# kakaobrain/hqtransformer

Measured on AMD Instinct MI355X. Metric: images/sec (256x256 class-cond sampling), higher is better.
Workload: dtype bf16

## Files before the change

hqtransformer_amd/csrc/split_ring.h:

```cpp
#pragma once
#include "split_kernels.h"
#include "split_device.h"

typedef _Float16 half8 __attribute__((ext_vector_type(8)));
typedef __attribute__((ext_vector_type(16))) float f32x16;
typedef __attribute__((ext_vector_type(4))) float f32x4;
typedef __attribute__((ext_vector_type(4))) unsigned int u32x4;

namespace {
constexpr float R_INV = 1.0f / 2048.0f;
constexpr int R_TY = 8, R_TX = 16, R_PITCH = R_TX + 2;
constexpr int R_ROWS = (R_TY + 2) * R_PITCH;
constexpr int R_PIECES = (R_ROWS + 15) / 16;
constexpr int R_PPW = 2 * R_PIECES / 4;
constexpr int R_CPITCH = 128 * 4 + 16;
static_assert(R_PPW == 6, "one piece per wave at taps 0..5");
constexpr int G_PITCH = 80, G_PLANE = 16 * R_PIECES * G_PITCH, G_LDS = 4 * G_PLANE;
static_assert(64 * R_CPITCH <= G_LDS, "epilogue staging (64 pixels at a time) must fit in the patch buffers");
static_assert(3 * G_PLANE + 38 * G_PITCH + 32 < 65536, "ds_read immediate offsets");

constexpr int H_RING = 3, H_AHEAD = H_RING - 1, H_STEPS = 18;
static_assert(H_STEPS % H_RING == 0, "static ring slots");
constexpr bool h_piece_at(int u) { u = ((u % H_STEPS) + H_STEPS) % H_STEPS; return (u % 9) < 6; }
constexpr int h_younger(int s, int per_step = 4) {
    int n = per_step * (H_AHEAD - 1);
    for (int u = s - H_AHEAD; u < s; ++u) n += h_piece_at(u) ? 1 : 0;
    return n;
}

__device__ __forceinline__ void r_xcd_tile(int& tile_m, int& tile_n, int panel) {
    const int nx = gridDim.x, total = gridDim.x * gridDim.y;
    int id = blockIdx.x + nx * blockIdx.y;
    if ((total & 7) == 0) id = (id & 7) * (total >> 3) + (id >> 3);
    if (panel > 0) {
        const int per = panel * nx, p = id / per, r = id - p * per;
        const int rows = min(panel, (int)gridDim.y - p * panel);
        tile_n = r / rows;
        tile_m = p * panel + (r - tile_n * rows);
        return;
    }
    tile_m = id / nx;
    tile_n = id - tile_m * nx;
}

__device__ __forceinline__ void ring_tile(int tile_m, int H, int W, int& img, int& trem, int& ty0, int& tx0, int& tiles_x, int& tiles_y) {
    tiles_x = W / R_TX; tiles_y = H / R_TY;
    img = tile_m / (tiles_x * tiles_y);
    trem = tile_m - img * (tiles_x * tiles_y);
    ty0 = (trem / tiles_x) * R_TY; tx0 = (trem % tiles_x) * R_TX;
}

typedef int ring_rsrc_t __attribute__((ext_vector_type(4)));
__device__ __forceinline__ ring_rsrc_t ring_image_rsrc(const void* A, int img, int Hin, int Win, int Cin) {
    const unsigned long long ib = (unsigned long long)(size_t)(reinterpret_cast<const half_t*>(A) + (long long)img * Hin * Win * (2 * Cin));
    ring_rsrc_t rsrc;
    rsrc[0] = __builtin_amdgcn_readfirstlane((int)(unsigned)ib);
    rsrc[1] = __builtin_amdgcn_readfirstlane((int)(unsigned)(ib >> 32) & 0xffff);
    rsrc[2] = __builtin_amdgcn_readfirstlane(Hin * Win * 2 * Cin * 2);
    rsrc[3] = 0x00020000;
    return rsrc;
}
__device__ __forceinline__ void ring_piece_offsets(unsigned (&poff)[3], int wave, int lane, int ty0, int tx0, int H, int W, int Win, int up, int Cin) {
#pragma unroll
    for (int u = 0; u < 3; ++u) {
        const int piece = wave + 4 * u;
        const int q = piece * 16 + (lane >> 2);
        const int qy = (q * 3641) >> 16, qx = q - qy * R_PITCH;
        const int iy = ty0 + qy - 1, ix = tx0 + qx - 1;
        const bool in = (q < R_ROWS) & ((unsigned)iy < (unsigned)H) & ((unsigned)ix < (unsigned)W);
        const unsigned off = (unsigned)((((iy >> up) * Win + (ix >> up)) * (2 * Cin) + (lane & 3) * 8) * 2);
        poff[u] = in ? off : 0x80000000u;
    }
}
__device__ __forceinline__ unsigned ring_piece_base(unsigned lds_base, int wave, int lane) {
    return lds_base + wave * (16 * G_PITCH) + (lane >> 2) * G_PITCH + (lane & 3) * 16;
}
__device__ __forceinline__ unsigned ring_frag_base(unsigned lds_base, int row, int fk) { return lds_base + row * G_PITCH + fk * 16; }

__device__ __forceinline__ void ring_load_piece(u32x4& dst, const unsigned (&poff)[3], const ring_rsrc_t& rsrc, int c, int u, int Cin) {
    asm volatile("buffer_load_dwordx4 %0, %1, %2, %3 offen" : "=v"(dst) : "v"(poff[u % 3]), "s"(rsrc), "s"(c * 64 + (u / 3) * Cin * 2));
}
__device__ __forceinline__ void ring_store_piece(unsigned piece_base, const u32x4& src, int buf, int u) {
    asm volatile("ds_write_b128 %0, %1 offset:%2" :: "v"(piece_base), "v"(src), "n"((buf * 2 + u / 3) * G_PLANE + 4 * (u % 3) * 16 * G_PITCH) : "memory");
}
__device__ __forceinline__ void ring_read_a16(half8 (&ah)[4], half8 (&al)[4], unsigned abase, int ps, int tapoff, int i, int slot) {
    asm volatile("ds_read_b128 %0, %1 offset:%2" : "=v"(ah[slot]) : "v"(abase), "n"(ps * 2 * G_PLANE + (i * R_PITCH + tapoff) * G_PITCH));
    asm volatile("ds_read_b128 %0, %1 offset:%2" : "=v"(al[slot]) : "v"(abase), "n"(ps * 2 * G_PLANE + (i * R_PITCH + tapoff) * G_PITCH + G_PLANE));
}
__device__ __forceinline__ void ring_read_a16(half8 (&ah)[4], half8 (&al)[4], unsigned abase, int ps, int tapoff, int i) {
    ring_read_a16(ah, al, abase, ps, tapoff, i, i % 4);
}
__device__ __forceinline__ void ring_load_b4(half8 (&wh)[2], half8 (&wl)[2], unsigned lane16, const char* bfrag, long long S) {
    const char* p = bfrag + S * 4096;
    asm volatile("global_load_dwordx4 %0, %1, %2" : "=v"(wh[0]) : "v"(lane16), "s"(p));
    asm volatile("global_load_dwordx4 %0, %1, %2 offset:1024" : "=v"(wl[0]) : "v"(lane16), "s"(p));
    asm volatile("global_load_dwordx4 %0, %1, %2 offset:2048" : "=v"(wh[1]) : "v"(lane16), "s"(p));
    asm volatile("global_load_dwordx4 %0, %1, %2 offset:3072" : "=v"(wl[1]) : "v"(lane16), "s"(p));
}
__device__ __forceinline__ void ring_load_b2(half8& wh, half8& wl, unsigned lane16, const char* bfrag, long long S) {
    const char* p = bfrag + S * 4096;
    asm volatile("global_load_dwordx4 %0, %1, %2" : "=v"(wh) : "v"(lane16), "s"(p));
    asm volatile("global_load_dwordx4 %0, %1, %2 offset:1024" : "=v"(wl) : "v"(lane16), "s"(p));
}

template <class V, int NI, int NJ>
__device__ __forceinline__ void ring_sink_acc(const GemmArgs& g, const V (&accm)[NI][NJ], const V (&accx)[NI][NJ]) {
    float sacc = 0.0f;
#pragma unroll
    for (int i = 0; i < NI; ++i)
#pragma unroll
        for (int j = 0; j < NJ; ++j)
#pragma unroll
            for (int r = 0; r < (int)(sizeof(V) / sizeof(float)); ++r) sacc += accm[i][j][r] + accx[i][j][r];
    if (sacc == 12345.678f) reinterpret_cast<float*>(g.C)[0] = sacc;
}

__device__ __forceinline__ void ring_bias8(const GemmArgs& g, int nn, float (&bv)[8]) {
#pragma unroll
    for (int e = 0; e < 8; ++e) bv[e] = (g.bias && nn + e < g.N) ? g.bias[nn + e] : 0.0f;
}
template <int PASSES, bool OUT_SPLIT, class PixelOf>
__device__ __forceinline__ void ring_store_rows(const GemmArgs& g, const char* stage, int tid, int n0, const float (&bv)[8], bool active,
                                                PixelOf pixel_of, float (&gs)[8], float (&gq)[8], bool& bad) {
    float* Cb = reinterpret_cast<float*>(g.C);
    const float* Rb = reinterpret_cast<const float*>(g.resid);
    const int c8 = (tid & 15) * 8, nn = n0 + c8;
    if (active && nn < g.N) {
        long long moff[PASSES];
        f32x4 r0[PASSES], r1[PASSES];
#pragma unroll
        for (int pass = 0; pass < PASSES; ++pass) {
            const int r = pass * 16 + (tid >> 4);
            moff[pass] = pixel_of(r) * g.ldc + nn;
            if (Rb) { r0[pass] = *reinterpret_cast<const f32x4*>(Rb + moff[pass]); r1[pass] = *reinterpret_cast<const f32x4*>(Rb + moff[pass] + 4); }
        }
#pragma unroll
        for (int pass = 0; pass < PASSES; ++pass) {
            const int r = pass * 16 + (tid >> 4);
            const f32x4 lo = *reinterpret_cast<const f32x4*>(stage + r * R_CPITCH + c8 * 4);
            const f32x4 hi = *reinterpret_cast<const f32x4*>(stage + r * R_CPITCH + c8 * 4 + 16);
            float v[8] = {lo[0], lo[1], lo[2], lo[3], hi[0], hi[1], hi[2], hi[3]};
#pragma unroll
            for (int e = 0; e < 8; ++e) v[e] = v[e] * g.alpha + bv[e];
            if (Rb) {
#pragma unroll
                for (int e = 0; e < 4; ++e) { v[e] += r0[pass][e]; v[4 + e] += r1[pass][e]; }
            }
            if (OUT_SPLIT && g.out_split) {
                unsigned hi[4], lo[4];
                split8_checked(v, hi, lo, bad);
                half_t* P = reinterpret_cast<half_t*>(g.C) + 2 * moff[pass] - nn;
                *reinterpret_cast<u32x4*>(P) = u32x4{hi[0], hi[1], hi[2], hi[3]};
                *reinterpret_cast<u32x4*>(P + g.N) = u32x4{lo[0], lo[1], lo[2], lo[3]};
            } else {
                const f32x4 o0 = {v[0], v[1], v[2], v[3]}, o1 = {v[4], v[5], v[6], v[7]};
                *reinterpret_cast<f32x4*>(Cb + moff[pass]) = o0;
                *reinterpret_cast<f32x4*>(Cb + moff[pass] + 4) = o1;
            }
            if (g.gn_part_out_d) {
#pragma clang fp contract(off)
#pragma unroll
                for (int e = 0; e < 8; ++e) { gs[e] += v[e]; const float sq = v[e] * v[e]; gq[e] += sq; }
            }
        }
    }
}
template <int PASSES, class PixelOf>
__device__ __forceinline__ void ring_store_rows(const GemmArgs& g, const char* stage, int tid, int n0, const float (&bv)[8], bool active,
                                                PixelOf pixel_of, float (&gs)[8], float (&gq)[8]) {
    bool bad = false;
    ring_store_rows<PASSES, false>(g, stage, tid, n0, bv, active, pixel_of, gs, gq, bad);
}
__device__ __forceinline__ void ring_reduce_gn(const GemmArgs& g, char* lds_raw, int tid, const float (&gs)[8], const float (&gq)[8], int n0,
                                               bool active, long long part) {
    if (!g.gn_part_out_d) return;
    const int c8 = (tid & 15) * 8;
    __syncthreads();
    float* redw = reinterpret_cast<float*>(lds_raw);
    if (active) {
#pragma unroll
        for (int e = 0; e < 8; ++e) {
            redw[(((tid >> 4) * 128) + c8 + e) * 2] = gs[e];
            redw[(((tid >> 4) * 128) + c8 + e) * 2 + 1] = gq[e];
        }
    }
    __syncthreads();
    const float* red = reinterpret_cast<const float*>(lds_raw);
    if (active && tid < 128) {
        double sa = 0.0, sq = 0.0;
#pragma unroll
        for (int rg = 0; rg < 16; ++rg) { sa += (double)red[((rg * 128) + tid) * 2]; sq += (double)red[((rg * 128) + tid) * 2 + 1]; }
        const int cpg = g.N / g.gn_out_groups;
        for (int off = cpg >> 1; off > 0; off >>= 1) { sa += __shfl_xor(sa, off, 64); sq += __shfl_xor(sq, off, 64); }
        const int ch = n0 + tid;
        if (ch < g.N && (tid & (cpg - 1)) == 0) {
            double* pp = g.gn_part_out_d + (part * g.gn_out_groups + ch / cpg) * 2;
            pp[0] = sa; pp[1] = sq;
        }
    }
}
}
```

hqtransformer_amd/csrc/split_stream_conv.hip:

```cpp
#include "split_kernels.h"
#include "split_ring.h"
#include "gemm_generic.h"
#include <algorithm>
#include <cstdlib>
#include <type_traits>

constexpr size_t R_FRAG_PAD = 3 * 4 * 512;
size_t split_frag_elems(int N, int Cin) { return (size_t)((N + 31) / 32) * (Cin / 32) * 9 * 4 * 512 + R_FRAG_PAD; }

__global__ void pack_split_frag16_kernel(const float* __restrict__ w, half_t* __restrict__ out, int N, int Cin, size_t total) {
    const int NC = Cin / 32;
    for (size_t i = blockIdx.x * (size_t)blockDim.x + threadIdx.x; i < total; i += (size_t)gridDim.x * blockDim.x) {
        const int j = (int)(i & 7), lane = (int)((i >> 3) & 63);
        size_t ch = i >> 9;
        const int plane = (int)(ch & 1); ch >>= 1;
        const int blk = (int)(ch & 1); ch >>= 1;
        const int tap = (int)(ch % 9); ch /= 9;
        const int c = (int)(ch % NC);
        const int t = (int)(ch / NC);
        const int n = t * 32 + blk * 16 + (lane & 15), k = tap * Cin + c * 32 + 8 * (lane >> 4) + j;
        const float x = n < N ? w[(size_t)n * 9 * Cin + k] : 0.0f;
        const half_t hi = (half_t)x;
        out[i] = plane ? (half_t)((x - (float)hi) * 2048.0f) : hi;
    }
}
hipError_t launch_pack_split_frag16(const float* w_tapmajor, half_t* out, int N, int Cin, hipStream_t st) {
    const size_t total = split_frag_elems(N, Cin) - R_FRAG_PAD;
    pack_split_frag16_kernel<<<(int)std::min<size_t>((total + 255) / 256, 8192), 256, 0, st>>>(w_tapmajor, out, N, Cin, total);
    return hipGetLastError();
}

namespace {
__device__ __forceinline__ void h_stage_half(char* stage, const f32x4 (&accm)[8][2], const f32x4 (&accx)[8][2], int half, int wave, int fx, int fk) {
#pragma unroll
    for (int ii = 0; ii < 4; ++ii) {
        const int i = half * 4 + ii, r = ii * 16 + fx;
#pragma unroll
        for (int j = 0; j < 2; ++j) {
            const int nl = wave * 32 + j * 16 + 4 * fk;
            f32x4 v;
#pragma unroll
            for (int e = 0; e < 4; ++e) v[e] = accm[i][j][e] + accx[i][j][e] * R_INV;
            *reinterpret_cast<f32x4*>(stage + r * R_CPITCH + nl * 4) = v;
        }
    }
}
}

template <int ABL = 0>
__global__ __launch_bounds__(256, 2) void conv3x3_split_ring16_kernel(GemmArgs g) {
    constexpr int NI = 8;
    extern __shared__ __attribute__((aligned(16))) char lds_raw[];
    const unsigned lds_base = (unsigned)(size_t)(__attribute__((address_space(3))) char*)lds_raw;
    const int tid = threadIdx.x, lane = tid & 63;
    const int wave = __builtin_amdgcn_readfirstlane(tid >> 6);
    const int fx = lane & 15, fk = lane >> 4;
    int tile_m, tile_n;
    r_xcd_tile(tile_m, tile_n, g.tile_panel);
    const int n0 = tile_n * 128;
    int img, trem, ty0, tx0, tiles_x, tiles_y;
    ring_tile(tile_m, g.H, g.W, img, trem, ty0, tx0, tiles_x, tiles_y);
    const int Hin = g.H >> g.upsample, Win = g.W >> g.upsample;
    const int NC = g.Cin / 32;

    const ring_rsrc_t img_rsrc = ring_image_rsrc(g.A, img, Hin, Win, g.Cin);
    unsigned poff[3];
    ring_piece_offsets(poff, wave, lane, ty0, tx0, g.H, g.W, Win, g.upsample, g.Cin);
    u32x4 pst[2];
    unsigned piece_base = ring_piece_base(lds_base, wave, lane);

    const char* bfrag = reinterpret_cast<const char*>(reinterpret_cast<const half_t*>(g.Bw_frag16) + (size_t)(n0 / 32 + wave) * ((size_t)NC * 9 * 2048));
    unsigned lane16 = lane * 16;

    f32x4 accm[NI][2], accx[NI][2];
#pragma unroll
    for (int i = 0; i < NI; ++i)
#pragma unroll
        for (int j = 0; j < 2; ++j)
#pragma unroll
            for (int r = 0; r < 4; ++r) { accm[i][j][r] = 0.0f; accx[i][j][r] = 0.0f; }
    const unsigned abase = ring_frag_base(lds_base, fx, fk);
    half8 ah[4], al[4];
    half8 wh[H_RING][2], wl[H_RING][2];

#pragma unroll
    for (int rnd = 0; rnd < 3; ++rnd) {
        ring_load_piece(pst[0], poff, img_rsrc, 0, 2 * rnd, g.Cin); ring_load_piece(pst[1], poff, img_rsrc, 0, 2 * rnd + 1, g.Cin);
        asm volatile("s_waitcnt vmcnt(0)" : "+v"(pst[0]), "+v"(pst[1]));
        ring_store_piece(piece_base, pst[0], 0, 2 * rnd); ring_store_piece(piece_base, pst[1], 0, 2 * rnd + 1);
    }
#pragma unroll
    for (int s = 0; s < H_AHEAD; ++s) ring_load_b4(wh[s], wl[s], lane16, bfrag, s);
    asm volatile("s_waitcnt vmcnt(0) lgkmcnt(0)" ::: "memory");

#pragma unroll 1
    for (int c0 = 0; c0 < NC; c0 += 2) {
#pragma unroll
        for (int cc = 0; cc < 2; ++cc) {
            const int c = c0 + cc, cn = min(c + 1, NC - 1);
            __builtin_amdgcn_s_barrier();
            __builtin_amdgcn_sched_barrier(0);
            if (ABL != 4) { ring_read_a16(ah, al, abase, cc, 0, 0); ring_read_a16(ah, al, abase, cc, 0, 1); ring_read_a16(ah, al, abase, cc, 0, 2); ring_read_a16(ah, al, abase, cc, 0, 3); }
#pragma unroll
            for (int tap = 0; tap < 9; ++tap) {
                const int s = cc * 9 + tap, slot = s % H_RING, nslot = (s + H_AHEAD) % H_RING;
                const long long S = (long long)c0 * 9 + s;
                const int tapoff = (tap / 3) * R_PITCH + tap % 3, ntapoff = ((tap + 1) / 3) * R_PITCH + (tap + 1) % 3;
                if (ABL != 4) asm volatile("s_waitcnt vmcnt(%4)" : "+v"(wh[slot][0]), "+v"(wl[slot][0]), "+v"(wh[slot][1]), "+v"(wl[slot][1]) : "n"(h_younger(s)));
#pragma unroll
                for (int pr = 0; pr < 4; ++pr) {
                    const int i0 = 2 * pr, i1 = 2 * pr + 1;
                    if (ABL != 4) {
                        const bool more = !(tap == 8 && pr == 3);
                        if (more) asm volatile("s_waitcnt lgkmcnt(4)" : "+v"(ah[i0 % 4]), "+v"(al[i0 % 4]), "+v"(ah[i1 % 4]), "+v"(al[i1 % 4]));
                        else asm volatile("s_waitcnt lgkmcnt(0)" : "+v"(ah[i0 % 4]), "+v"(al[i0 % 4]), "+v"(ah[i1 % 4]), "+v"(al[i1 % 4]));
                    }
#pragma unroll
                    for (int ii = 0; ii < 2; ++ii)
#pragma unroll
                        for (int j = 0; j < 2; ++j)
                            accm[i0 + ii][j] = __builtin_amdgcn_mfma_f32_16x16x32_f16(wh[slot][j], ah[(i0 + ii) % 4], accm[i0 + ii][j], 0, 0, 0);
#pragma unroll
                    for (int ii = 0; ii < 2; ++ii)
#pragma unroll
                        for (int j = 0; j < 2; ++j)
                            accx[i0 + ii][j] = __builtin_amdgcn_mfma_f32_16x16x32_f16(wh[slot][j], al[(i0 + ii) % 4], accx[i0 + ii][j], 0, 0, 0);
#pragma unroll
                    for (int ii = 0; ii < 2; ++ii)
#pragma unroll
                        for (int j = 0; j < 2; ++j)
                            accx[i0 + ii][j] = __builtin_amdgcn_mfma_f32_16x16x32_f16(wl[slot][j], ah[(i0 + ii) % 4], accx[i0 + ii][j], 0, 0, 0);
                    if (ABL == 4) continue;
                    if (pr < 2) {
                        if (pr == 0) { ring_read_a16(ah, al, abase, cc, tapoff, 4); ring_read_a16(ah, al, abase, cc, tapoff, 5); }
                        else { ring_read_a16(ah, al, abase, cc, tapoff, 6); ring_read_a16(ah, al, abase, cc, tapoff, 7); }
                    } else if (tap < 8) {
                        if (pr == 2) { ring_read_a16(ah, al, abase, cc, ntapoff, 0); ring_read_a16(ah, al, abase, cc, ntapoff, 1); }
                        else { ring_read_a16(ah, al, abase, cc, ntapoff, 2); ring_read_a16(ah, al, abase, cc, ntapoff, 3); }
                    }
                    if (pr == 0 && ABL != 5) ring_load_b4(wh[nslot], wl[nslot], lane16, bfrag, S + H_AHEAD);
                    if (pr == 1 && ABL != 2) {
                        if (tap >= 2 && tap - 2 < R_PPW) {
                            if (tap - 1 < R_PPW) asm volatile("s_waitcnt vmcnt(9)" : "+v"(pst[tap % 2]));
                            else asm volatile("s_waitcnt vmcnt(8)" : "+v"(pst[tap % 2]));
                            ring_store_piece(piece_base, pst[tap % 2], cc ^ 1, tap - 2);
                        }
                        if (tap < R_PPW) ring_load_piece(pst[tap % 2], poff, img_rsrc, cn, tap, g.Cin);
                    }
                }
            }
        }
    }
    asm volatile("s_waitcnt vmcnt(0) lgkmcnt(0)" ::: "memory");
    __builtin_amdgcn_s_barrier();
    __builtin_amdgcn_sched_barrier(0);
    if (ABL == 1) { ring_sink_acc(g, accm, accx); return; }
    const long long pix0 = ((long long)img * g.H + ty0) * g.W + tx0;
    char* stage = lds_raw;
    float bv[8], gs[8], gq[8];
    ring_bias8(g, n0 + (tid & 15) * 8, bv);
    bool bad = false;
#pragma unroll
    for (int e = 0; e < 8; ++e) { gs[e] = 0.0f; gq[e] = 0.0f; }
#pragma unroll
    for (int half = 0; half < 2; ++half) {
        if (half > 0) __syncthreads();
        h_stage_half(stage, accm, accx, half, wave, fx, fk);
        __syncthreads();
        ring_store_rows<4, true>(g, stage, tid, n0, bv, true, [&](int r) { return pix0 + (long long)(half * 4 + (r >> 4)) * g.W + (r & 15); }, gs, gq, bad);
    }
    if (bad && g.range_flag) atomicOr(g.range_flag, 1);
    ring_reduce_gn(g, lds_raw, tid, gs, gq, n0, true, (long long)img * (tiles_x * tiles_y) + trem);
}


__global__ void pack_split_up16_kernel(const float* __restrict__ w, half_t* __restrict__ out, int N, int Cin, size_t total) {
    const int NC = Cin / 32, NG = (N + 31) / 32;
    for (size_t i = blockIdx.x * (size_t)blockDim.x + threadIdx.x; i < total; i += (size_t)gridDim.x * blockDim.x) {
        const int j = (int)(i & 7), lane = (int)((i >> 3) & 63);
        size_t ch = i >> 9;
        const int plane = (int)(ch & 1); ch >>= 1;
        const int blk = (int)(ch & 1); ch >>= 1;
        const int tap = (int)(ch & 3); ch >>= 2;
        const int c = (int)(ch % NC); ch /= NC;
        const int t = (int)(ch % NG);
        const int phase = (int)(ch / NG);
        const int pa = phase >> 1, pb = phase & 1, ty = tap >> 1, tx = tap & 1;
        const int n = t * 32 + blk * 16 + (lane & 15), kin = c * 32 + 8 * (lane >> 4) + j;
        const int ky0 = pa == 0 ? (ty == 0 ? 0 : 1) : (ty == 0 ? 0 : 2), ky1 = pa == 0 ? (ty == 0 ? 0 : 2) : (ty == 0 ? 1 : 2);
        const int kx0 = pb == 0 ? (tx == 0 ? 0 : 1) : (tx == 0 ? 0 : 2), kx1 = pb == 0 ? (tx == 0 ? 0 : 2) : (tx == 0 ? 1 : 2);
        double x = 0.0;
        if (n < N)
            for (int ky = ky0; ky <= ky1; ++ky)
                for (int kx = kx0; kx <= kx1; ++kx) x += (double)w[(size_t)n * 9 * Cin + (size_t)(ky * 3 + kx) * Cin + kin];
        const half_t hi = (half_t)(float)x;
        out[i] = plane ? (half_t)(float)((x - (double)(float)hi) * 2048.0) : hi;
    }
}
size_t split_up_elems(int N, int Cin) { return (size_t)4 * ((N + 31) / 32) * (Cin / 32) * 4 * 2048 + 2048; }
hipError_t launch_pack_split_up16(const float* w_tapmajor, half_t* out, int N, int Cin, hipStream_t st) {
    const size_t total = split_up_elems(N, Cin) - 2048;
    pack_split_up16_kernel<<<(int)std::min<size_t>((total + 255) / 256, 8192), 256, 0, st>>>(w_tapmajor, out, N, Cin, total);
    return hipGetLastError();
}

template <int ABL = 0>
__global__ __launch_bounds__(256, 2) void conv2x2_split_up16_kernel(GemmArgs g) {
    constexpr int NI = 8, TAPS = 4;
    extern __shared__ __attribute__((aligned(16))) char lds_raw[];
    const unsigned lds_base = (unsigned)(size_t)(__attribute__((address_space(3))) char*)lds_raw;
    const int tid = threadIdx.x, lane = tid & 63;
    const int wave = __builtin_amdgcn_readfirstlane(tid >> 6);
    const int fx = lane & 15, fk = lane >> 4;
    int tile_m, tile_v;
    r_xcd_tile(tile_m, tile_v, g.tile_panel);
    const int NT = g.N / 128;
    const int phase = tile_v / NT, pa = phase >> 1, pb = phase & 1;
    const int n0 = (tile_v - phase * NT) * 128;
    const int Hin = g.H >> 1, Win = g.W >> 1;
    int img, trem, ty0, tx0, tiles_x, tiles_y;
    ring_tile(tile_m, Hin, Win, img, trem, ty0, tx0, tiles_x, tiles_y);
    const int NC = g.Cin / 32;

    const ring_rsrc_t img_rsrc = ring_image_rsrc(g.A, img, Hin, Win, g.Cin);
    unsigned poff[3];
    ring_piece_offsets(poff, wave, lane, ty0, tx0, Hin, Win, Win, 0, g.Cin);
    u32x4 pst[R_PPW];
    unsigned piece_base = ring_piece_base(lds_base, wave, lane);

    const char* bfrag = reinterpret_cast<const char*>(reinterpret_cast<const half_t*>(g.Bw_up16) +
                                                      ((size_t)phase * (g.N / 32) + n0 / 32 + wave) * ((size_t)NC * TAPS * 2048));
    unsigned lane16 = lane * 16;

    f32x4 accm[NI][2], accx[NI][2];
#pragma unroll
    for (int i = 0; i < NI; ++i)
#pragma unroll
        for (int j = 0; j < 2; ++j)
#pragma unroll
            for (int r = 0; r < 4; ++r) { accm[i][j][r] = 0.0f; accx[i][j][r] = 0.0f; }
    const unsigned abase = ring_frag_base(lds_base, fx + pa * R_PITCH + pb, fk);
    half8 ah[4], al[4];
    half8 wh[2][2], wl[2][2];

#pragma unroll
    for (int u = 0; u < R_PPW; ++u) ring_load_piece(pst[u], poff, img_rsrc, 0, u, g.Cin);
    asm volatile("s_waitcnt vmcnt(0)" : "+v"(pst[0]), "+v"(pst[1]), "+v"(pst[2]), "+v"(pst[3]), "+v"(pst[4]), "+v"(pst[5]));
#pragma unroll
    for (int u = 0; u < R_PPW; ++u) ring_store_piece(piece_base, pst[u], 0, u);
    ring_load_b4(wh[0], wl[0], lane16, bfrag, 0);
    asm volatile("s_waitcnt vmcnt(0) lgkmcnt(0)" ::: "memory");

#pragma unroll 1
    for (int c0 = 0; c0 < NC; c0 += 2) {
#pragma unroll
        for (int cc = 0; cc < 2; ++cc) {
            const int c = c0 + cc, cn = min(c + 1, NC - 1);
            __builtin_amdgcn_s_barrier();
            __builtin_amdgcn_sched_barrier(0);
            if (ABL != 4) { ring_read_a16(ah, al, abase, cc, 0, 0); ring_read_a16(ah, al, abase, cc, 0, 1); ring_read_a16(ah, al, abase, cc, 0, 2); ring_read_a16(ah, al, abase, cc, 0, 3); }
#pragma unroll
            for (int tap = 0; tap < TAPS; ++tap) {
                const int s = cc * TAPS + tap, slot = s % 2, nslot = (s + 1) % 2;
                const long long S = (long long)c0 * TAPS + s;
                const int tapoff = (tap / 2) * R_PITCH + tap % 2, ntapoff = ((tap + 1) / 2) * R_PITCH + (tap + 1) % 2;
                if (ABL != 4) {
                    if (tap == 1 || tap == 2) asm volatile("s_waitcnt vmcnt(3)" : "+v"(wh[slot][0]), "+v"(wl[slot][0]), "+v"(wh[slot][1]), "+v"(wl[slot][1]));
                    else asm volatile("s_waitcnt vmcnt(0)" : "+v"(wh[slot][0]), "+v"(wl[slot][0]), "+v"(wh[slot][1]), "+v"(wl[slot][1]));
                    if (ABL != 5) ring_load_b4(wh[nslot], wl[nslot], lane16, bfrag, S + 1);
                }
#pragma unroll
                for (int pr = 0; pr < 4; ++pr) {
                    const int i0 = 2 * pr, i1 = 2 * pr + 1;
                    if (ABL != 4) {
                        const bool more = !(tap == TAPS - 1 && pr == 3);
                        if (more) asm volatile("s_waitcnt lgkmcnt(4)" : "+v"(ah[i0 % 4]), "+v"(al[i0 % 4]), "+v"(ah[i1 % 4]), "+v"(al[i1 % 4]));
                        else asm volatile("s_waitcnt lgkmcnt(0)" : "+v"(ah[i0 % 4]), "+v"(al[i0 % 4]), "+v"(ah[i1 % 4]), "+v"(al[i1 % 4]));
                    }
#pragma unroll
                    for (int ii = 0; ii < 2; ++ii)
#pragma unroll
                        for (int j = 0; j < 2; ++j)
                            accm[i0 + ii][j] = __builtin_amdgcn_mfma_f32_16x16x32_f16(wh[slot][j], ah[(i0 + ii) % 4], accm[i0 + ii][j], 0, 0, 0);
#pragma unroll
                    for (int ii = 0; ii < 2; ++ii)
#pragma unroll
                        for (int j = 0; j < 2; ++j)
                            accx[i0 + ii][j] = __builtin_amdgcn_mfma_f32_16x16x32_f16(wh[slot][j], al[(i0 + ii) % 4], accx[i0 + ii][j], 0, 0, 0);
#pragma unroll
                    for (int ii = 0; ii < 2; ++ii)
#pragma unroll
                        for (int j = 0; j < 2; ++j)
                            accx[i0 + ii][j] = __builtin_amdgcn_mfma_f32_16x16x32_f16(wl[slot][j], ah[(i0 + ii) % 4], accx[i0 + ii][j], 0, 0, 0);
                    if (ABL == 4) continue;
                    if (pr >= 1 && tap >= 2 && ABL != 2) {
                        const int u = 3 * (tap - 2) + pr - 1;
                        if (tap == 2) asm volatile("s_waitcnt vmcnt(7)" : "+v"(pst[u])); else asm volatile("s_waitcnt vmcnt(4)" : "+v"(pst[u]));
                        ring_store_piece(piece_base, pst[u], cc ^ 1, u);
                    }
                    if (pr < 2) {
                        if (pr == 0) { ring_read_a16(ah, al, abase, cc, tapoff, 4); ring_read_a16(ah, al, abase, cc, tapoff, 5); }
                        else { ring_read_a16(ah, al, abase, cc, tapoff, 6); ring_read_a16(ah, al, abase, cc, tapoff, 7); }
                    } else if (tap < TAPS - 1) {
                        if (pr == 2) { ring_read_a16(ah, al, abase, cc, ntapoff, 0); ring_read_a16(ah, al, abase, cc, ntapoff, 1); }
                        else { ring_read_a16(ah, al, abase, cc, ntapoff, 2); ring_read_a16(ah, al, abase, cc, ntapoff, 3); }
                    }
                    if (pr >= 1 && tap < 2 && ABL != 2) ring_load_piece(pst[3 * tap + pr - 1], poff, img_rsrc, cn, 3 * tap + pr - 1, g.Cin);
                }
            }
        }
    }
    asm volatile("s_waitcnt vmcnt(0) lgkmcnt(0)" ::: "memory");
    __builtin_amdgcn_s_barrier();
    __builtin_amdgcn_sched_barrier(0);
    if (ABL == 1) { ring_sink_acc(g, accm, accx); return; }
    char* stage = lds_raw;
    float bv[8], gs[8], gq[8];
    ring_bias8(g, n0 + (tid & 15) * 8, bv);
#pragma unroll
    for (int e = 0; e < 8; ++e) { gs[e] = 0.0f; gq[e] = 0.0f; }
#pragma unroll
    for (int half = 0; half < 2; ++half) {
        if (half > 0) __syncthreads();
        h_stage_half(stage, accm, accx, half, wave, fx, fk);
        __syncthreads();
        ring_store_rows<4>(g, stage, tid, n0, bv, true, [&](int r) {
            const long long oy = 2 * (ty0 + half * 4 + (r >> 4)) + pa, ox = 2 * (tx0 + (r & 15)) + pb;
            return ((long long)img * g.H + oy) * g.W + ox;
        }, gs, gq);
    }
    ring_reduce_gn(g, lds_raw, tid, gs, gq, n0, true, ((long long)img * (tiles_x * tiles_y) + trem) * 4 + phase);
}


__global__ __launch_bounds__(256, 2) void conv3x3_split_out16_kernel(GemmArgs g) {
    extern __shared__ __attribute__((aligned(16))) char lds_raw[];
    const unsigned lds_base = (unsigned)(size_t)(__attribute__((address_space(3))) char*)lds_raw;
    const int tid = threadIdx.x, lane = tid & 63;
    const int wave = __builtin_amdgcn_readfirstlane(tid >> 6);
    const int fx = lane & 15, fk = lane >> 4;
    const int tile_m = blockIdx.y;
    int img, trem, ty0, tx0, tiles_x, tiles_y;
    ring_tile(tile_m, g.H, g.W, img, trem, ty0, tx0, tiles_x, tiles_y);
    const int Hin = g.H >> g.upsample, Win = g.W >> g.upsample;
    const int NC = g.Cin / 32;

    const ring_rsrc_t img_rsrc = ring_image_rsrc(g.A, img, Hin, Win, g.Cin);
    unsigned poff[3];
    ring_piece_offsets(poff, wave, lane, ty0, tx0, g.H, g.W, Win, g.upsample, g.Cin);
    u32x4 pst[2];
    unsigned piece_base = ring_piece_base(lds_base, wave, lane);

    const char* bfrag = reinterpret_cast<const char*>(g.Bw_frag16);
    unsigned lane16 = lane * 16;

    f32x4 accm[2], accx[2];
#pragma unroll
    for (int i = 0; i < 2; ++i)
#pragma unroll
        for (int r = 0; r < 4; ++r) { accm[i][r] = 0.0f; accx[i][r] = 0.0f; }
    const unsigned abase = ring_frag_base(lds_base, 2 * wave * R_PITCH + fx, fk);
    half8 ah[4], al[4];
    half8 wh[H_RING], wl[H_RING];

#pragma unroll
    for (int rnd = 0; rnd < 3; ++rnd) {
        ring_load_piece(pst[0], poff, img_rsrc, 0, 2 * rnd, g.Cin); ring_load_piece(pst[1], poff, img_rsrc, 0, 2 * rnd + 1, g.Cin);
        asm volatile("s_waitcnt vmcnt(0)" : "+v"(pst[0]), "+v"(pst[1]));
        ring_store_piece(piece_base, pst[0], 0, 2 * rnd); ring_store_piece(piece_base, pst[1], 0, 2 * rnd + 1);
    }
#pragma unroll
    for (int s = 0; s < H_AHEAD; ++s) ring_load_b2(wh[s], wl[s], lane16, bfrag, s);
    asm volatile("s_waitcnt vmcnt(0) lgkmcnt(0)" ::: "memory");

#pragma unroll 1
    for (int c0 = 0; c0 < NC; c0 += 2) {
#pragma unroll
        for (int cc = 0; cc < 2; ++cc) {
            const int c = c0 + cc, cn = min(c + 1, NC - 1);
            __builtin_amdgcn_s_barrier();
            __builtin_amdgcn_sched_barrier(0);
            ring_read_a16(ah, al, abase, cc, 0, 0, 0); ring_read_a16(ah, al, abase, cc, 0, 1, 1);
#pragma unroll
            for (int tap = 0; tap < 9; ++tap) {
                const int s = cc * 9 + tap, slot = s % H_RING, nslot = (s + H_AHEAD) % H_RING;
                const long long S = (long long)c0 * 9 + s;
                const int par = tap & 1;
                const int ntapoff = ((tap + 1) / 3) * R_PITCH + (tap + 1) % 3;
                if (tap < 8) {
                    if (par == 0) { ring_read_a16(ah, al, abase, cc, ntapoff, 0, 2); ring_read_a16(ah, al, abase, cc, ntapoff, 1, 3); }
                    else { ring_read_a16(ah, al, abase, cc, ntapoff, 0, 0); ring_read_a16(ah, al, abase, cc, ntapoff, 1, 1); }
                }
                asm volatile("s_waitcnt vmcnt(%2)" : "+v"(wh[slot]), "+v"(wl[slot]) : "n"(h_younger(s, 2)));
                if (tap < 8) asm volatile("s_waitcnt lgkmcnt(4)" : "+v"(ah[2 * par]), "+v"(al[2 * par]), "+v"(ah[2 * par + 1]), "+v"(al[2 * par + 1]));
                else asm volatile("s_waitcnt lgkmcnt(0)" : "+v"(ah[2 * par]), "+v"(al[2 * par]), "+v"(ah[2 * par + 1]), "+v"(al[2 * par + 1]));
                accm[0] = __builtin_amdgcn_mfma_f32_16x16x32_f16(wh[slot], ah[2 * par], accm[0], 0, 0, 0);
                accm[1] = __builtin_amdgcn_mfma_f32_16x16x32_f16(wh[slot], ah[2 * par + 1], accm[1], 0, 0, 0);
                accx[0] = __builtin_amdgcn_mfma_f32_16x16x32_f16(wh[slot], al[2 * par], accx[0], 0, 0, 0);
                accx[1] = __builtin_amdgcn_mfma_f32_16x16x32_f16(wh[slot], al[2 * par + 1], accx[1], 0, 0, 0);
                accx[0] = __builtin_amdgcn_mfma_f32_16x16x32_f16(wl[slot], ah[2 * par], accx[0], 0, 0, 0);
                accx[1] = __builtin_amdgcn_mfma_f32_16x16x32_f16(wl[slot], ah[2 * par + 1], accx[1], 0, 0, 0);
                ring_load_b2(wh[nslot], wl[nslot], lane16, bfrag, S + H_AHEAD);
                if (tap >= 2 && tap - 2 < R_PPW) {
                    if (tap - 1 < R_PPW) asm volatile("s_waitcnt vmcnt(5)" : "+v"(pst[tap % 2]));
                    else asm volatile("s_waitcnt vmcnt(4)" : "+v"(pst[tap % 2]));
                    ring_store_piece(piece_base, pst[tap % 2], cc ^ 1, tap - 2);
                }
                if (tap < R_PPW) ring_load_piece(pst[tap % 2], poff, img_rsrc, cn, tap, g.Cin);
            }
        }
    }
    asm volatile("s_waitcnt vmcnt(0) lgkmcnt(0)" ::: "memory");
    float* Cb = reinterpret_cast<float*>(g.C);
    const long long hw = (long long)g.H * g.W;
#pragma unroll
    for (int i = 0; i < 2; ++i) {
        const long long pix = (long long)(ty0 + 2 * wave + i) * g.W + tx0 + fx;
#pragma unroll
        for (int r = 0; r < 4; ++r) {
            const int n = 4 * fk + r;
            if (n >= g.N) continue;
            float v = (accm[i][r] + accx[i][r] * R_INV) * g.alpha + (g.bias ? g.bias[n] : 0.0f);
            if (g.clamp01) v = fminf(fmaxf(0.5f * v + 0.5f, 0.0f), 1.0f);
            Cb[((long long)img * g.N + n) * hw + pix] = v;
        }
    }
}

bool split_conv3_emits_planes(const GemmArgs& g) {
    static const bool off = getenv("HQT_SPLIT_PLANES_OUT") && atoi(getenv("HQT_SPLIT_PLANES_OUT")) == 0;
    return !off && split_stream_ok(g) && g.store == STORE_ROWS && !g.upsample && g.ldc == g.N && g.N % 8 == 0;
}
bool split_stream_ok(const GemmArgs& g) {
    if (!g.Bw_frag16) return false;
    if (g.H % R_TY != 0 || g.W % R_TX != 0 || g.Cin % 64 != 0) return false;
    if ((long long)(g.H >> g.upsample) * (g.W >> g.upsample) * g.Cin * 4 >= (1ll << 31)) return false;
    if (g.store == STORE_NCHW) return g.N <= 16;
    return g.N % 128 == 0 && g.ldc % 8 == 0;
}
static bool split_up_shape(const GemmArgs& g) {
    static const bool off = getenv("HQT_SPLIT_UP") && atoi(getenv("HQT_SPLIT_UP")) == 0;
    return !off && g.upsample == 1 && g.Bw_up16 && g.store == STORE_ROWS && (g.H / 2) % R_TY == 0 && (g.W / 2) % R_TX == 0 && g.N % 128 == 0;
}
int split_stream_tiles_per_image(const GemmArgs& g) { return split_up_shape(g) ? 4 * (g.H / 2 / R_TY) * (g.W / 2 / R_TX) : (g.H / R_TY) * (g.W / R_TX); }
hipError_t launch_split_conv3_stream(const GemmArgs& g, hipStream_t st) {
    if (g.store == STORE_NCHW) conv3x3_split_out16_kernel<<<dim3(1, g.M / (R_TY * R_TX), 1), 256, G_LDS, st>>>(g);
    else if (split_up_shape(g)) conv2x2_split_up16_kernel<0><<<dim3(4 * (g.N / 128), g.M / 4 / (R_TY * R_TX), 1), 256, G_LDS, st>>>(g);
    else conv3x3_split_ring16_kernel<0><<<dim3(g.N / 128, g.M / (R_TY * R_TX), 1), 256, G_LDS, st>>>(g);
    return hipGetLastError();
}
hipError_t split_stream_configure() {
    hipError_t e = hipFuncSetAttribute(reinterpret_cast<const void*>(conv3x3_split_ring16_kernel<0>), hipFuncAttributeMaxDynamicSharedMemorySize, G_LDS);
    if (e != hipSuccess) return e;
    e = hipFuncSetAttribute(reinterpret_cast<const void*>(conv2x2_split_up16_kernel<0>), hipFuncAttributeMaxDynamicSharedMemorySize, G_LDS);
    if (e != hipSuccess) return e;
    return hipFuncSetAttribute(reinterpret_cast<const void*>(conv3x3_split_out16_kernel), hipFuncAttributeMaxDynamicSharedMemorySize, G_LDS);
}

namespace {
constexpr int O_T = 16, O_P = O_T + 2, O_CH = 32, O_PITCH = O_CH + 4;
constexpr int O_LDS = O_P * O_P * O_PITCH * 4;
constexpr int O_V4 = O_P * O_P * (O_CH / 4);
constexpr int O_PER = (O_V4 + 255) / 256;
typedef __attribute__((ext_vector_type(2))) float f32x2;
}

template <int NO>
__global__ __launch_bounds__(256, 3) void conv_out_direct_kernel(GemmArgs g) {
    extern __shared__ __attribute__((aligned(16))) char lds_raw[];
    float* patch = reinterpret_cast<float*>(lds_raw);
    const int tid = threadIdx.x;
    const int tiles_x = g.W / O_T, tiles = tiles_x * (g.H / O_T);
    const int img = blockIdx.x / tiles, trem = blockIdx.x - img * tiles;
    const int ty0 = (trem / tiles_x) * O_T, tx0 = (trem % tiles_x) * O_T;
    const int C = g.Cin, NC = C / O_CH;
    const float* __restrict__ X = reinterpret_cast<const float*>(g.A) + (long long)img * g.H * g.W * C;
    const float* __restrict__ Wt = reinterpret_cast<const float*>(g.Bw);
    const int v = tid & 7;
    int src[O_PER];
    unsigned inside = 0;
#pragma unroll
    for (int u = 0; u < O_PER; ++u) {
        const int q = (tid + 256 * u) >> 3;
        const int qy = q / O_P, qx = q - qy * O_P;
        const int iy = ty0 + qy - 1, ix = tx0 + qx - 1;
        const bool in = (q < O_P * O_P) & ((unsigned)iy < (unsigned)g.H) & ((unsigned)ix < (unsigned)g.W);
        src[u] = in ? (iy * g.W + ix) * C + v * 4 : v * 4;
        inside |= in ? 1u << u : 0u;
    }
    const int cpg = C / g.gn_groups;
    const float* stats = g.gn_stats + (long long)img * g.gn_groups * 2;
    f32x4 r[O_PER];
    auto fetch = [&](int c) {
#pragma unroll
        for (int u = 0; u < O_PER; ++u) r[u] = *reinterpret_cast<const f32x4*>(X + src[u] + c * O_CH);
    };
    auto fill = [&](int c) {
        float a[4], b[4];
#pragma unroll
        for (int j = 0; j < 4; ++j) {
            const int ch = c * O_CH + v * 4 + j;
            const float mu = stats[(ch / cpg) * 2], rs = stats[(ch / cpg) * 2 + 1];
            a[j] = rs * g.gn_gamma[ch];
            b[j] = g.gn_beta[ch] - mu * a[j];
        }
#pragma unroll
        for (int u = 0; u < O_PER; ++u) {
            const int slot = tid + 256 * u;
            if (slot >= O_V4) continue;
            f32x4 y = {0.0f, 0.0f, 0.0f, 0.0f};
            if (inside >> u & 1) {
#pragma unroll
                for (int j = 0; j < 4; ++j) {
                    float t = r[u][j] * a[j] + b[j];
                    if (g.gn_swish) t = t * __builtin_amdgcn_rcpf(1.0f + __expf(-t));
                    y[j] = t;
                }
            }
            *reinterpret_cast<f32x4*>(patch + (slot >> 3) * O_PITCH + v * 4) = y;
        }
    };
    const int py = tid >> 4, px = tid & 15;
    f32x2 acc[NO];
#pragma unroll
    for (int o = 0; o < NO; ++o) acc[o] = f32x2{0.0f, 0.0f};
    fetch(0);
    for (int c = 0; c < NC; ++c) {
        if (c > 0) __syncthreads();
        fill(c);
        __syncthreads();
        if (c + 1 < NC) fetch(c + 1);
#pragma unroll
        for (int tap = 0; tap < 9; ++tap) {
            const float* row = patch + ((py + tap / 3) * O_P + px + tap % 3) * O_PITCH;
            f32x4 x[O_CH / 4];
#pragma unroll
            for (int q = 0; q < O_CH / 4; ++q) x[q] = *reinterpret_cast<const f32x4*>(row + q * 4);
#pragma unroll
            for (int o = 0; o < NO; ++o) {
                const float* w = Wt + ((long long)o * 9 + tap) * C + c * O_CH;
#pragma unroll
                for (int q = 0; q < O_CH / 4; ++q) {
                    acc[o] += f32x2{x[q][0], x[q][1]} * f32x2{w[q * 4], w[q * 4 + 1]};
                    acc[o] += f32x2{x[q][2], x[q][3]} * f32x2{w[q * 4 + 2], w[q * 4 + 3]};
                }
            }
        }
    }
    float* Cb = reinterpret_cast<float*>(g.C);
    const long long hw = (long long)g.H * g.W, pix = (long long)(ty0 + py) * g.W + tx0 + px;
#pragma unroll
    for (int o = 0; o < NO; ++o) {
        float val = (acc[o][0] + acc[o][1]) * g.alpha + (g.bias ? g.bias[o] : 0.0f);
        if (g.clamp01) val = fminf(fmaxf(0.5f * val + 0.5f, 0.0f), 1.0f);
        Cb[((long long)img * NO + o) * hw + pix] = val;
    }
}

bool conv_out_direct_ok(const GemmArgs& g) {
    static const bool off = getenv("HQT_CONV_OUT_DIRECT") && atoi(getenv("HQT_CONV_OUT_DIRECT")) == 0;
    return !off && g.conv_taps == 9 && g.store == STORE_NCHW && g.N >= 1 && g.N <= 4 && g.Cin % O_CH == 0 && g.H % O_T == 0 && g.W % O_T == 0 &&
           !g.upsample && !g.conv_stride2 && !g.resid && g.gn_stats && g.gn_groups > 0 && g.Cin % g.gn_groups == 0 &&
           (long long)g.H * g.W * g.Cin < (1ll << 31);
}
hipError_t launch_conv_out_direct(const GemmArgs& g, hipStream_t st) {
    const int grid = (g.M / (g.H * g.W)) * (g.H / O_T) * (g.W / O_T);
    switch (g.N) {
        case 1: conv_out_direct_kernel<1><<<grid, 256, O_LDS, st>>>(g); break;
        case 2: conv_out_direct_kernel<2><<<grid, 256, O_LDS, st>>>(g); break;
        case 3: conv_out_direct_kernel<3><<<grid, 256, O_LDS, st>>>(g); break;
        default: conv_out_direct_kernel<4><<<grid, 256, O_LDS, st>>>(g); break;
    }
    return hipGetLastError();
}
```

Before: 1710.

## Overlap conv prologue loads and prefetch residual rows before epilogue barrier

Issues all image-piece loads and the first weight-fragment loads together in the conv kernel prologues. Each piece is stored to LDS behind a graded vmcnt wait instead of serialized rounds that wait for everything, and accumulator zeroing is placed between issue and wait. The epilogue now fetches residual rows before the final barrier and prefetches the second half's residuals while the first half is staged, with the residual/no-residual choice made at compile time. Clock64 timestamp instrumentation is added behind an ablation template value, which raises register pressure and depends on correct hand-counted vmcnt values.

```diff
diff --git a/hqtransformer_amd/csrc/split_ring.h b/hqtransformer_amd/csrc/split_ring.h
--- a/hqtransformer_amd/csrc/split_ring.h
+++ b/hqtransformer_amd/csrc/split_ring.h
@@ -115,28 +115,47 @@
     if (sacc == 12345.678f) reinterpret_cast<float*>(g.C)[0] = sacc;
 }
 
+__device__ __forceinline__ void ring_write_stamps(const GemmArgs& g, int tid, const long long (&stamp)[3]) {
+    asm volatile("s_waitcnt vmcnt(0)" ::: "memory");
+    const long long now = clock64();
+    if (tid == 0) {
+        long long* d = reinterpret_cast<long long*>(g.am_best) + (size_t)(blockIdx.x + gridDim.x * blockIdx.y) * 4;
+        d[0] = stamp[0]; d[1] = stamp[1]; d[2] = stamp[2]; d[3] = now;
+    }
+}
+
 __device__ __forceinline__ void ring_bias8(const GemmArgs& g, int nn, float (&bv)[8]) {
 #pragma unroll
     for (int e = 0; e < 8; ++e) bv[e] = (g.bias && nn + e < g.N) ? g.bias[nn + e] : 0.0f;
 }
-template <int PASSES, bool OUT_SPLIT, class PixelOf>
-__device__ __forceinline__ void ring_store_rows(const GemmArgs& g, const char* stage, int tid, int n0, const float (&bv)[8], bool active,
-                                                PixelOf pixel_of, float (&gs)[8], float (&gq)[8], bool& bad) {
+template <int PASSES, bool SURE = false, class PixelOf>
+__device__ __forceinline__ void ring_fetch_rows(const GemmArgs& g, int tid, int n0, bool active, PixelOf pixel_of, f32x4 (&r0)[PASSES],
+                                                f32x4 (&r1)[PASSES]) {
+    const float* Rb = reinterpret_cast<const float*>(g.resid);
+    const int nn = n0 + (tid & 15) * 8;
+    const bool fetch = SURE || (Rb && active && nn < g.N);
+#pragma unroll
+    for (int pass = 0; pass < PASSES; ++pass) {
+        f32x4 a = {0.0f, 0.0f, 0.0f, 0.0f}, b = a;
+        if (fetch) {
+            const long long moff = pixel_of(pass * 16 + (tid >> 4)) * g.ldc + nn;
+            a = *reinterpret_cast<const f32x4*>(Rb + moff); b = *reinterpret_cast<const f32x4*>(Rb + moff + 4);
+        }
+        r0[pass] = a; r1[pass] = b;
+    }
+}
+template <int PASSES, bool OUT_SPLIT, bool SURE = false, class PixelOf>
+__device__ __forceinline__ void ring_store_fetched(const GemmArgs& g, const char* stage, int tid, int n0, const float (&bv)[8], bool active,
+                                                   PixelOf pixel_of, const f32x4 (&r0)[PASSES], const f32x4 (&r1)[PASSES],
+                                                   float (&gs)[8], float (&gq)[8], bool& bad) {
     float* Cb = reinterpret_cast<float*>(g.C);
     const float* Rb = reinterpret_cast<const float*>(g.resid);
     const int c8 = (tid & 15) * 8, nn = n0 + c8;
-    if (active && nn < g.N) {
-        long long moff[PASSES];
-        f32x4 r0[PASSES], r1[PASSES];
+    if (SURE || (active && nn < g.N)) {
 #pragma unroll
         for (int pass = 0; pass < PASSES; ++pass) {
             const int r = pass * 16 + (tid >> 4);
-            moff[pass] = pixel_of(r) * g.ldc + nn;
-            if (Rb) { r0[pass] = *reinterpret_cast<const f32x4*>(Rb + moff[pass]); r1[pass] = *reinterpret_cast<const f32x4*>(Rb + moff[pass] + 4); }
-        }
-#pragma unroll
-        for (int pass = 0; pass < PASSES; ++pass) {
-            const int r = pass * 16 + (tid >> 4);
+            const long long moff = pixel_of(r) * g.ldc + nn;
             const f32x4 lo = *reinterpret_cast<const f32x4*>(stage + r * R_CPITCH + c8 * 4);
             const f32x4 hi = *reinterpret_cast<const f32x4*>(stage + r * R_CPITCH + c8 * 4 + 16);
             float v[8] = {lo[0], lo[1], lo[2], lo[3], hi[0], hi[1], hi[2], hi[3]};
@@ -149,13 +168,13 @@
             if (OUT_SPLIT && g.out_split) {
                 unsigned hi[4], lo[4];
                 split8_checked(v, hi, lo, bad);
-                half_t* P = reinterpret_cast<half_t*>(g.C) + 2 * moff[pass] - nn;
+                half_t* P = reinterpret_cast<half_t*>(g.C) + 2 * moff - nn;
                 *reinterpret_cast<u32x4*>(P) = u32x4{hi[0], hi[1], hi[2], hi[3]};
                 *reinterpret_cast<u32x4*>(P + g.N) = u32x4{lo[0], lo[1], lo[2], lo[3]};
             } else {
                 const f32x4 o0 = {v[0], v[1], v[2], v[3]}, o1 = {v[4], v[5], v[6], v[7]};
-                *reinterpret_cast<f32x4*>(Cb + moff[pass]) = o0;
-                *reinterpret_cast<f32x4*>(Cb + moff[pass] + 4) = o1;
+                *reinterpret_cast<f32x4*>(Cb + moff) = o0;
+                *reinterpret_cast<f32x4*>(Cb + moff + 4) = o1;
             }
             if (g.gn_part_out_d) {
 #pragma clang fp contract(off)
@@ -164,6 +183,13 @@
             }
         }
     }
+}
+template <int PASSES, bool OUT_SPLIT, class PixelOf>
+__device__ __forceinline__ void ring_store_rows(const GemmArgs& g, const char* stage, int tid, int n0, const float (&bv)[8], bool active,
+                                                PixelOf pixel_of, float (&gs)[8], float (&gq)[8], bool& bad) {
+    f32x4 r0[PASSES], r1[PASSES];
+    ring_fetch_rows<PASSES, false>(g, tid, n0, active, pixel_of, r0, r1);
+    ring_store_fetched<PASSES, OUT_SPLIT, false>(g, stage, tid, n0, bv, active, pixel_of, r0, r1, gs, gq, bad);
 }
 template <int PASSES, class PixelOf>
 __device__ __forceinline__ void ring_store_rows(const GemmArgs& g, const char* stage, int tid, int n0, const float (&bv)[8], bool active,
diff --git a/hqtransformer_amd/csrc/split_stream_conv.hip b/hqtransformer_amd/csrc/split_stream_conv.hip
--- a/hqtransformer_amd/csrc/split_stream_conv.hip
+++ b/hqtransformer_amd/csrc/split_stream_conv.hip
@@ -50,6 +50,8 @@
 template <int ABL = 0>
 __global__ __launch_bounds__(256, 2) void conv3x3_split_ring16_kernel(GemmArgs g) {
     constexpr int NI = 8;
+    long long stamp[3];
+    if (ABL == 6) stamp[0] = clock64();
     extern __shared__ __attribute__((aligned(16))) char lds_raw[];
     const unsigned lds_base = (unsigned)(size_t)(__attribute__((address_space(3))) char*)lds_raw;
     const int tid = threadIdx.x, lane = tid & 63;
@@ -73,25 +75,33 @@
     unsigned lane16 = lane * 16;
 
     f32x4 accm[NI][2], accx[NI][2];
-#pragma unroll
-    for (int i = 0; i < NI; ++i)
-#pragma unroll
-        for (int j = 0; j < 2; ++j)
-#pragma unroll
-            for (int r = 0; r < 4; ++r) { accm[i][j][r] = 0.0f; accx[i][j][r] = 0.0f; }
     const unsigned abase = ring_frag_base(lds_base, fx, fk);
     half8 ah[4], al[4];
     half8 wh[H_RING][2], wl[H_RING][2];
 
-#pragma unroll
-    for (int rnd = 0; rnd < 3; ++rnd) {
-        ring_load_piece(pst[0], poff, img_rsrc, 0, 2 * rnd, g.Cin); ring_load_piece(pst[1], poff, img_rsrc, 0, 2 * rnd + 1, g.Cin);
-        asm volatile("s_waitcnt vmcnt(0)" : "+v"(pst[0]), "+v"(pst[1]));
-        ring_store_piece(piece_base, pst[0], 0, 2 * rnd); ring_store_piece(piece_base, pst[1], 0, 2 * rnd + 1);
-    }
-#pragma unroll
-    for (int s = 0; s < H_AHEAD; ++s) ring_load_b4(wh[s], wl[s], lane16, bfrag, s);
-    asm volatile("s_waitcnt vmcnt(0) lgkmcnt(0)" ::: "memory");
+    {
+        u32x4 pp[R_PPW];
+#pragma unroll
+        for (int u = 0; u < R_PPW; ++u) ring_load_piece(pp[u], poff, img_rsrc, 0, u, g.Cin);
+#pragma unroll
+        for (int s = 0; s < H_AHEAD; ++s) ring_load_b4(wh[s], wl[s], lane16, bfrag, s);
+        __builtin_amdgcn_sched_barrier(0);
+#pragma unroll
+        for (int i = 0; i < NI; ++i)
+#pragma unroll
+            for (int j = 0; j < 2; ++j)
+#pragma unroll
+                for (int r = 0; r < 4; ++r) { accm[i][j][r] = 0.0f; accx[i][j][r] = 0.0f; }
+        __builtin_amdgcn_sched_barrier(0);
+#pragma unroll
+        for (int u = 0; u < R_PPW; ++u) {
+            asm volatile("s_waitcnt vmcnt(%1)" : "+v"(pp[u]) : "n"(4 * H_AHEAD + R_PPW - 1 - u));
+            ring_store_piece(piece_base, pp[u], 0, u);
+        }
+    }
+    if (ABL == 4) asm volatile("s_waitcnt vmcnt(0)" ::: "memory");
+    asm volatile("s_waitcnt lgkmcnt(0)" ::: "memory");
+    if (ABL == 6) { stamp[1] = clock64(); __builtin_amdgcn_sched_barrier(0); }
 
 #pragma unroll 1
     for (int c0 = 0; c0 < NC; c0 += 2) {
@@ -152,25 +162,40 @@
         }
     }
     asm volatile("s_waitcnt vmcnt(0) lgkmcnt(0)" ::: "memory");
-    __builtin_amdgcn_s_barrier();
-    __builtin_amdgcn_sched_barrier(0);
-    if (ABL == 1) { ring_sink_acc(g, accm, accx); return; }
+    __builtin_amdgcn_s_waitcnt(0);
+    if (ABL == 6) { stamp[2] = clock64(); __builtin_amdgcn_sched_barrier(0); }
     const long long pix0 = ((long long)img * g.H + ty0) * g.W + tx0;
-    char* stage = lds_raw;
-    float bv[8], gs[8], gq[8];
-    ring_bias8(g, n0 + (tid & 15) * 8, bv);
-    bool bad = false;
-#pragma unroll
-    for (int e = 0; e < 8; ++e) { gs[e] = 0.0f; gq[e] = 0.0f; }
-#pragma unroll
-    for (int half = 0; half < 2; ++half) {
-        if (half > 0) __syncthreads();
-        h_stage_half(stage, accm, accx, half, wave, fx, fk);
-        __syncthreads();
-        ring_store_rows<4, true>(g, stage, tid, n0, bv, true, [&](int r) { return pix0 + (long long)(half * 4 + (r >> 4)) * g.W + (r & 15); }, gs, gq, bad);
-    }
-    if (bad && g.range_flag) atomicOr(g.range_flag, 1);
-    ring_reduce_gn(g, lds_raw, tid, gs, gq, n0, true, (long long)img * (tiles_x * tiles_y) + trem);
+    const int oW = g.W;
+    const auto pixel_of = [&](int half) { return [pix0, oW, half](int r) { return pix0 + (long long)(half * 4 + (r >> 4)) * oW + (r & 15); }; };
+    const auto epilogue = [&](auto with_resid) {
+        constexpr bool RES = decltype(with_resid)::value;
+        float bv[8], gs[8], gq[8];
+        f32x4 r0[2][4], r1[2][4];
+        if (ABL != 1) {
+            ring_bias8(g, n0 + (tid & 15) * 8, bv);
+            if (RES) ring_fetch_rows<4, true>(g, tid, n0, true, pixel_of(0), r0[0], r1[0]);
+            __builtin_amdgcn_sched_barrier(0);
+        }
+        __builtin_amdgcn_s_barrier();
+        __builtin_amdgcn_sched_barrier(0);
+        if (ABL == 1) { ring_sink_acc(g, accm, accx); return; }
+        char* stage = lds_raw;
+        bool bad = false;
+#pragma unroll
+        for (int e = 0; e < 8; ++e) { gs[e] = 0.0f; gq[e] = 0.0f; }
+#pragma unroll
+        for (int half = 0; half < 2; ++half) {
+            if (half > 0) __syncthreads();
+            h_stage_half(stage, accm, accx, half, wave, fx, fk);
+            if (RES && half == 0) ring_fetch_rows<4, true>(g, tid, n0, true, pixel_of(1), r0[1], r1[1]);
+            __syncthreads();
+            ring_store_fetched<4, true, true>(g, stage, tid, n0, bv, true, pixel_of(half), r0[half], r1[half], gs, gq, bad);
+        }
+        if (bad && g.range_flag) atomicOr(g.range_flag, 1);
+        ring_reduce_gn(g, lds_raw, tid, gs, gq, n0, true, (long long)img * (tiles_x * tiles_y) + trem);
+    };
+    if (g.resid) epilogue(std::true_type{}); else epilogue(std::false_type{});
+    if (ABL == 6) ring_write_stamps(g, tid, stamp);
 }
 
 
@@ -207,6 +232,8 @@
 template <int ABL = 0>
 __global__ __launch_bounds__(256, 2) void conv2x2_split_up16_kernel(GemmArgs g) {
     constexpr int NI = 8, TAPS = 4;
+    long long stamp[3];
+    if (ABL == 6) stamp[0] = clock64();
     extern __shared__ __attribute__((aligned(16))) char lds_raw[];
     const unsigned lds_base = (unsigned)(size_t)(__attribute__((address_space(3))) char*)lds_raw;
     const int tid = threadIdx.x, lane = tid & 63;
@@ -233,23 +260,29 @@
     unsigned lane16 = lane * 16;
 
     f32x4 accm[NI][2], accx[NI][2];
-#pragma unroll
-    for (int i = 0; i < NI; ++i)
-#pragma unroll
-        for (int j = 0; j < 2; ++j)
-#pragma unroll
-            for (int r = 0; r < 4; ++r) { accm[i][j][r] = 0.0f; accx[i][j][r] = 0.0f; }
     const unsigned abase = ring_frag_base(lds_base, fx + pa * R_PITCH + pb, fk);
     half8 ah[4], al[4];
     half8 wh[2][2], wl[2][2];
 
 #pragma unroll
     for (int u = 0; u < R_PPW; ++u) ring_load_piece(pst[u], poff, img_rsrc, 0, u, g.Cin);
-    asm volatile("s_waitcnt vmcnt(0)" : "+v"(pst[0]), "+v"(pst[1]), "+v"(pst[2]), "+v"(pst[3]), "+v"(pst[4]), "+v"(pst[5]));
-#pragma unroll
-    for (int u = 0; u < R_PPW; ++u) ring_store_piece(piece_base, pst[u], 0, u);
     ring_load_b4(wh[0], wl[0], lane16, bfrag, 0);
-    asm volatile("s_waitcnt vmcnt(0) lgkmcnt(0)" ::: "memory");
+    __builtin_amdgcn_sched_barrier(0);
+#pragma unroll
+    for (int i = 0; i < NI; ++i)
+#pragma unroll
+        for (int j = 0; j < 2; ++j)
+#pragma unroll
+            for (int r = 0; r < 4; ++r) { accm[i][j][r] = 0.0f; accx[i][j][r] = 0.0f; }
+    __builtin_amdgcn_sched_barrier(0);
+#pragma unroll
+    for (int u = 0; u < R_PPW; ++u) {
+        asm volatile("s_waitcnt vmcnt(%1)" : "+v"(pst[u]) : "n"(4 + R_PPW - 1 - u));
+        ring_store_piece(piece_base, pst[u], 0, u);
+    }
+    if (ABL == 4) asm volatile("s_waitcnt vmcnt(0)" ::: "memory");
+    asm volatile("s_waitcnt lgkmcnt(0)" ::: "memory");
+    if (ABL == 6) { stamp[1] = clock64(); __builtin_amdgcn_sched_barrier(0); }
 
 #pragma unroll 1
     for (int c0 = 0; c0 < NC; c0 += 2) {
@@ -311,25 +344,43 @@
         }
     }
     asm volatile("s_waitcnt vmcnt(0) lgkmcnt(0)" ::: "memory");
-    __builtin_amdgcn_s_barrier();
-    __builtin_amdgcn_sched_barrier(0);
-    if (ABL == 1) { ring_sink_acc(g, accm, accx); return; }
-    char* stage = lds_raw;
-    float bv[8], gs[8], gq[8];
-    ring_bias8(g, n0 + (tid & 15) * 8, bv);
-#pragma unroll
-    for (int e = 0; e < 8; ++e) { gs[e] = 0.0f; gq[e] = 0.0f; }
-#pragma unroll
-    for (int half = 0; half < 2; ++half) {
-        if (half > 0) __syncthreads();
-        h_stage_half(stage, accm, accx, half, wave, fx, fk);
-        __syncthreads();
-        ring_store_rows<4>(g, stage, tid, n0, bv, true, [&](int r) {
+    __builtin_amdgcn_s_waitcnt(0);
+    if (ABL == 6) { stamp[2] = clock64(); __builtin_amdgcn_sched_barrier(0); }
+    const int oH = g.H, oW = g.W;
+    const auto pixel_of = [&](int half) {
+        return [=](int r) {
             const long long oy = 2 * (ty0 + half * 4 + (r >> 4)) + pa, ox = 2 * (tx0 + (r & 15)) + pb;
-            return ((long long)img * g.H + oy) * g.W + ox;
-        }, gs, gq);
-    }
-    ring_reduce_gn(g, lds_raw, tid, gs, gq, n0, true, ((long long)img * (tiles_x * tiles_y) + trem) * 4 + phase);
+            return ((long long)img * oH + oy) * oW + ox;
+        };
+    };
+    const auto epilogue = [&](auto with_resid) {
+        constexpr bool RES = decltype(with_resid)::value;
+        float bv[8], gs[8], gq[8];
+        f32x4 r0[2][4], r1[2][4];
+        if (ABL != 1) {
+            ring_bias8(g, n0 + (tid & 15) * 8, bv);
+            if (RES) ring_fetch_rows<4, true>(g, tid, n0, true, pixel_of(0), r0[0], r1[0]);
+            __builtin_amdgcn_sched_barrier(0);
+        }
+        __builtin_amdgcn_s_barrier();
+        __builtin_amdgcn_sched_barrier(0);
+        if (ABL == 1) { ring_sink_acc(g, accm, accx); return; }
+        char* stage = lds_raw;
+        bool bad = false;
+#pragma unroll
+        for (int e = 0; e < 8; ++e) { gs[e] = 0.0f; gq[e] = 0.0f; }
+#pragma unroll
+        for (int half = 0; half < 2; ++half) {
+            if (half > 0) __syncthreads();
+            h_stage_half(stage, accm, accx, half, wave, fx, fk);
+            if (RES && half == 0) ring_fetch_rows<4, true>(g, tid, n0, true, pixel_of(1), r0[1], r1[1]);
+            __syncthreads();
+            ring_store_fetched<4, false, true>(g, stage, tid, n0, bv, true, pixel_of(half), r0[half], r1[half], gs, gq, bad);
+        }
+        ring_reduce_gn(g, lds_raw, tid, gs, gq, n0, true, ((long long)img * (tiles_x * tiles_y) + trem) * 4 + phase);
+    };
+    if (g.resid) epilogue(std::true_type{}); else epilogue(std::false_type{});
+    if (ABL == 6) ring_write_stamps(g, tid, stamp);
 }
 
 
@@ -363,15 +414,19 @@
     half8 ah[4], al[4];
     half8 wh[H_RING], wl[H_RING];
 
-#pragma unroll
-    for (int rnd = 0; rnd < 3; ++rnd) {
-        ring_load_piece(pst[0], poff, img_rsrc, 0, 2 * rnd, g.Cin); ring_load_piece(pst[1], poff, img_rsrc, 0, 2 * rnd + 1, g.Cin);
-        asm volatile("s_waitcnt vmcnt(0)" : "+v"(pst[0]), "+v"(pst[1]));
-        ring_store_piece(piece_base, pst[0], 0, 2 * rnd); ring_store_piece(piece_base, pst[1], 0, 2 * rnd + 1);
-    }
-#pragma unroll
-    for (int s = 0; s < H_AHEAD; ++s) ring_load_b2(wh[s], wl[s], lane16, bfrag, s);
-    asm volatile("s_waitcnt vmcnt(0) lgkmcnt(0)" ::: "memory");
+    {
+        u32x4 pp[R_PPW];
+#pragma unroll
+        for (int u = 0; u < R_PPW; ++u) ring_load_piece(pp[u], poff, img_rsrc, 0, u, g.Cin);
+#pragma unroll
+        for (int s = 0; s < H_AHEAD; ++s) ring_load_b2(wh[s], wl[s], lane16, bfrag, s);
+#pragma unroll
+        for (int u = 0; u < R_PPW; ++u) {
+            asm volatile("s_waitcnt vmcnt(%1)" : "+v"(pp[u]) : "n"(2 * H_AHEAD + R_PPW - 1 - u));
+            ring_store_piece(piece_base, pp[u], 0, u);
+        }
+    }
+    asm volatile("s_waitcnt lgkmcnt(0)" ::: "memory");
 
 #pragma unroll 1
     for (int c0 = 0; c0 < NC; c0 += 2) {
```

Result: no change. 1718 (median of 6 runs) (+0.5%).
